# Kuntz-Lab/interactive-rate-tendons

Hardware: AMD Instinct MI355X
Metric: FK+collision checks/sec (3-tendon, 256^3 voxel env) (higher is better)
Workload: dtype f64

## Files before the change

interactive-rate-tendons_amd/_lib.py:

```python
import ctypes as C
import os
import subprocess

_PKG = os.path.dirname(os.path.abspath(__file__))
_ROOT = os.path.dirname(_PKG)
LIB_PATH = os.environ.get("TENDON_HIP_LIB") or os.path.join(_PKG, "libtendon_hip.so")
SRC_DIR = os.path.join(_PKG, "csrc")
HEADER = os.path.join(_ROOT, "include", "tendon_hip.h")

TR_OK, TR_ERR_INVALID_ARG, TR_ERR_OUT_OF_RANGE, TR_ERR_DOMAIN, TR_ERR_LENGTH, TR_ERR_RUNTIME, \
    TR_ERR_HIP, TR_ERR_UNSUPPORTED = range(8)

TR_FLAG_CONVERGED, TR_FLAG_LENGTH_OK, TR_FLAG_NO_SELFCOL, TR_FLAG_NO_VOXCOL, TR_FLAG_DOMAIN = 1, 2, 4, 8, 16
TR_CHECKER_BACKBONE, TR_CHECKER_SPHERES = 0, 1
TR_PROFILE_SLOTS = 6
PROFILE_SLOT_NAMES = ("fk_rk4_batch", "backbone_voxel_sweep", "cached_blocks_vs_grid", "edge_helpers", "fk_sweep_fused", "fk_verdict")

ABI_SYMBOLS = (
    "tr_create", "tr_destroy", "tr_last_error", "tr_state_size", "tr_num_points", "tr_device",
    "tr_home_lengths", "tr_set_grid", "tr_set_checker", "tr_grid_add_spheres", "tr_grid_add_capsules", "tr_grid_remove_interior", "tr_grid_dilate",
    "tr_grid_dilate_sphere", "tr_get_grid", "tr_reserve", "tr_reserve_edges", "tr_fk_batch", "tr_fk_batch_dev", "tr_fk_batch_retraction_dev",
    "tr_validate_shapes_retraction_dev",
    "tr_validate_batch", "tr_validate_batch_dev", "tr_validate_shapes_dev", "tr_validate_edges", "tr_validate_edges_indexed", "tr_validate_edges_last_valid",
    "tr_validate_edges_discrete",
# ... 54 lines not shown


class OutOfRange(TendonHipError, IndexError):
    status = TR_ERR_OUT_OF_RANGE


class DomainError(TendonHipError, ArithmeticError):
    status = TR_ERR_DOMAIN


class LengthError(TendonHipError, ValueError):
    status = TR_ERR_LENGTH


class HipError(TendonHipError):
    status = TR_ERR_HIP


class Unsupported(TendonHipError, NotImplementedError):
    status = TR_ERR_UNSUPPORTED


_EXC = {TR_ERR_INVALID_ARG: InvalidArgument, TR_ERR_OUT_OF_RANGE: OutOfRange, TR_ERR_DOMAIN: DomainError,
        TR_ERR_LENGTH: LengthError, TR_ERR_RUNTIME: TendonHipError, TR_ERR_HIP: HipError,
        TR_ERR_UNSUPPORTED: Unsupported}


HIPCC_FLAGS = ["--offload-arch=gfx950", "-O3", "-std=c++17", "-ffp-contract=off", "-fPIC"]
OBJ_DIR = os.path.join(SRC_DIR, "_obj")


def _units():
    fk_deps = ["fk_inst.hip", "fk_launch.hpp", "fk_kernel.hpp", "fk_retract_kernel.hpp", "fused_kernel.hpp", "verdict_kernel.hpp",
               "sweep_kernel.hpp", "sphere_kernel.hpp", "tr_types.hpp"]
    roadmap_deps = ["roadmap.hip", "roadmap_kernel.hpp", "search_kernel.hpp", "handback_feed.hpp", "roadmap_infra_host.inc", "roadmap_astar_host.inc",
                    "roadmap_components_host.inc", "roadmap_search_host.inc", "roadmap_solve_host.inc", "roadmap_tips_host.inc", "tipq_kernel.hpp"]
    fk_only = ["fk_inst.hip", "fk_kernel.hpp", "fk_retract_kernel.hpp", "cache_merge.hip", "sample.hip", "edge_queue_kernel.hpp"] + roadmap_deps
    main_deps = [f for f in os.listdir(SRC_DIR) if not f.startswith("_") and f not in fk_only]
    u = [("tendon_hip.o", "tendon_hip.hip", [], main_deps + [HEADER]),
         ("cache_merge.o", "cache_merge.hip", [], ["cache_merge.hip", "cache_merge.hpp"]),
         ("roadmap.o", "roadmap.hip", ["-pthread"], roadmap_deps + [HEADER]),
         ("sample.o", "sample.hip", [], ["sample.hip", "sample.hpp", "tr_types.hpp"])]
    q_deps = fk_deps + ["edge_queue_kernel.hpp", "edge_kernel.hpp"]
    for n in range(1, 9):
        for kind, tag in ((0, "u"), (1, "r"), (2, "f"), (3, "v"), (4, "w"), (5, "q")):
            u.append(("fk_%s%d.o" % (tag, n), "fk_inst.hip", ["-DTRK_INST_N=%d" % n, "-DTRK_INST_KIND=%d" % kind],
                      q_deps if kind == 5 else fk_deps))
    return u


def _sources():
    return [os.path.join(SRC_DIR, f) for f in sorted(os.listdir(SRC_DIR)) if not f.startswith("_")] + [HEADER]


def source_hash():
    import hashlib
    h = hashlib.sha1()
    for f in _sources():
        h.update(os.path.basename(f).encode())
        h.update(open(f, "rb").read())
    return h.hexdigest()[:16]


def build(force=False, verbose=False, jobs=None):
    stamp = LIB_PATH + ".srchash"
    want = source_hash()
    if not force and os.path.exists(LIB_PATH) and os.path.exists(stamp) and open(stamp).read().strip() == want:
# ... 189 lines not shown
```

interactive-rate-tendons_amd/csrc/edge_queue_kernel.hpp:

```cpp
#pragma once
#include "verdict_kernel.hpp"
#define TRK_EDGE_DEVICE_ONLY
#include "edge_kernel.hpp"

namespace trk {

__device__ __forceinline__ uint32_t eq_load(const uint32_t *p) { return __hip_atomic_load(p, __ATOMIC_RELAXED, __HIP_MEMORY_SCOPE_AGENT); }
__device__ __forceinline__ void eq_wait_vm() { asm volatile("s_waitcnt vmcnt(0)" ::: "memory"); }
__device__ __forceinline__ void eq_release() {
  eq_wait_vm();
  __builtin_amdgcn_fence(__ATOMIC_RELEASE, "agent");
  eq_wait_vm();
}
__device__ __forceinline__ void eq_acquire() {
  __builtin_amdgcn_fence(__ATOMIC_ACQUIRE, "agent");
  eq_wait_vm();
}
__device__ __forceinline__ int eq_bcast(int v) { return __builtin_amdgcn_readfirstlane(v); }
struct EqClock {
  unsigned long long t;
  __device__ __forceinline__ void start() { t = wall_clock64(); }
  __device__ __forceinline__ void lap(uint32_t *ctl, int word) {
    const unsigned long long n = wall_clock64();
    if (threadIdx.x == 0) __hip_atomic_fetch_add((unsigned long long *)(ctl + word), n - t, __ATOMIC_RELAXED, __HIP_MEMORY_SCOPE_AGENT);
// ... 150 lines not shown
    }
    ps.template sig_finish<false>();
    ps.finish();
    while (ps.qcount > 0) ps.flush();
    __syncthreads();
    LaneVerdict lv;
    int e2, h2, cnt2;
    {
      const VerdictArgs a = *va;
      const int sb = eq_stash_base(a.NM);
      e2 = VL_I(sb + lane); h2 = VL_I(sb + 64); cnt2 = VL_I(sb + 65);
      clk.t = (unsigned long long)VL_U(sb + 66) | ((unsigned long long)VL_U(sb + 67) << 32);
      lv = verdict_decide<N, false, true>(a, fl_, lane < cnt2);
    }
    const bool live2 = lane < cnt2;
    int zero2 = 0;
    asm volatile("" : "+s"(zero2));
    const EdgeQueueArgs &q2 = qa[zero2];
#ifdef TRK_EQ_TRACE
    const uint32_t tr_start = (uint32_t)clk.t;
    const unsigned long long tr_w0 = wall_clock64(), tr_c0 = (unsigned long long)clock64();
    { float x = (float)lane; for (int i = 0; i < 2000; i++) x = __builtin_fmaf(x, 1.0000001f, 0.5f); if (x == 12345.678f) asm volatile("s_nop 0"); }
    const unsigned long long tr_w1 = wall_clock64(), tr_c1 = (unsigned long long)clock64();
    const uint32_t tr_mhz = tr_w1 > tr_w0 ? (uint32_t)((tr_c1 - tr_c0) * 100ull / (tr_w1 - tr_w0)) : 0u;
#endif
    clk.lap(q2.ctl, EQ_T_FK);
#ifdef TRK_EQ_TRACE
    const uint32_t tr_fk = (uint32_t)clk.t;
#endif
    if (__any(lv.pending)) {
      __syncthreads();
      const double *st2 = q2.states + ((int64_t)h2 - (int64_t)blockIdx.x * 64) * K.state_size;
      const int64_t n2 = (int64_t)blockIdx.x * 64 + cnt2;
      fk_uniform_body<N, ROT, false, false>(st2, n2, q2.fb_ld, K, tab, steps, nsteps, q2.fb_out, NoPointHook(), nullptr, nullptr);
      __syncthreads();
      const FusedSweepArgs fa = *sa;
      bool exact = false;
      sweep_body<false>(q2.fb_in, n2, q2.fb_ld, fa.P, fa.CH, fa.NM, K, fa.g, fa.grid, fa.near_grid, 1, fa.debug, nullptr, nullptr, nullptr, &exact);
      __syncthreads();
      const uint32_t npend = (uint32_t)__popcll(__ballot(lv.pending));
      if (lane == 0) __hip_atomic_fetch_add(q2.ctl + EQ_PENDING, npend, __ATOMIC_RELAXED, __HIP_MEMORY_SCOPE_AGENT);
      if (lv.pending) lv.valid = exact;
      clk.lap(q2.ctl, EQ_T_EXACT);
    }

    if (live2 && !lv.valid) q2.edge_ok[e2] = 0u;
    eq_release();
    int old = 0;
    if (live2) old = __hip_atomic_fetch_add(q2.remaining + e2, -1, __ATOMIC_RELAXED, __HIP_MEMORY_SCOPE_AGENT);
    bool fin = live2 && old == 1;
    bool stop = false;
    EqClock sub = clk;
    sub.lap(q2.ctl, EQ_T_F0);
    if (__any(fin)) {
      eq_acquire();
      {
        const uint32_t nfin = (uint32_t)__popcll(__ballot(fin));
        if (lane == 0) __hip_atomic_fetch_add(q2.ctl + EQ_FINISHED, nfin, __ATOMIC_RELAXED, __HIP_MEMORY_SCOPE_AGENT);
      }
      int base_l = 0, ncand_l = 0;
      double rel_l = 0.0;
      if (fin && q2.edge_ok[e2] != 0u) {
        base_l = q2.lvl_base[e2]; ncand_l = q2.lvl_cnt[e2]; rel_l = q2.rel[e2];
        if (2 * ncand_l > EQ_MAX_CAND) {
          __hip_atomic_fetch_or(q2.ctl + EQ_FLAGS, EQF_DEEP, __ATOMIC_RELAXED, __HIP_MEMORY_SCOPE_AGENT);
          ncand_l = 0; stop = true;
        }
// ... 140 lines not shown
```

interactive-rate-tendons_amd/csrc/fk_kernel.hpp:

```cpp
#pragma once
#include <type_traits>
#include <hip/hip_runtime.h>
#include "tr_types.hpp"

namespace trk {

#ifndef TRK_NEWTON_STEPS
#define TRK_NEWTON_STEPS 1
#endif
__device__ __forceinline__ double fast_rcp(double x) {
  double y = __builtin_amdgcn_rcp(x);
  double e = __builtin_fma(-x, y, 1.0);
  y = __builtin_fma(e, y, y);
#if TRK_NEWTON_STEPS > 1
  e = __builtin_fma(-x, y, 1.0);
  y = __builtin_fma(e, y, y);
#endif
  return y;
}
__device__ __forceinline__ double fast_rsqrt(double x) {
  double y = __builtin_amdgcn_rsq(x);
  double hx = 0.5 * x;
  double t = __builtin_fma(-hx * y, y, 0.5);
  y = __builtin_fma(y, t, y);
#if TRK_NEWTON_STEPS > 1
  t = __builtin_fma(-hx * y, y, 0.5);
  y = __builtin_fma(y, t, y);
#endif
  return y;
}

template <int N, class Route>
__device__ __forceinline__ void strain_rates_routed(const double v[3], const double u[3], const double (&tau)[N],
                                                    Route &&route, const RobotK &K,
                                                    double dv[3], double du[3], double (&sdot)[N]) {
#pragma clang fp contract(fast)
  double Axx = K.ks0, Axy = 0, Axz = 0, Ayy = K.ks0, Ayz = 0, Azz = K.ks2, Z = 0;
  double B00 = 0, B01 = 0, B02 = 0, B10 = 0, B11 = 0, B12 = 0, B20 = 0, B21 = 0, B22 = 0, Q1 = 0, Q2 = 0;
  double Hxx = K.kb0, Hxy = 0, Hxz = 0, Hyy = K.kb0, Hyz = 0, Hzz = K.kb2;
  double ax = 0, ay = 0, az = 0, bx = 0, by = 0, bz = 0;
#pragma unroll
  for (int j = 0; j < N; j++) {
    double r6[6];
    route(j, r6);
    const double rx = r6[0], ry = r6[1];
    const double rdx = r6[2], rdy = r6[3];
    const double rddx = r6[4], rddy = r6[5];
    const double pdx = (v[0] + rdx) - u[2] * ry;
    const double pdy = (v[1] + rdy) + u[2] * rx;
    const double pdz = __builtin_fma(u[0], ry, __builtin_fma(-u[1], rx, v[2]));
    const double sxy = pdx * pdx + pdy * pdy, s2 = sxy + pdz * pdz;
    const double rs = fast_rsqrt(s2);
    sdot[j] = s2 * rs;
    const double cs2 = -tau[j] * rs;
    const double c = cs2 * (rs * rs);
    const double qx = c * pdx, qy = c * pdy, qz = c * pdz;
    Axx += qx * pdx; Axy += qx * pdy; Axz += qx * pdz; Ayy += qy * pdy; Ayz += qy * pdz; Azz += qz * pdz;
    Z += cs2;
    const double ez = rx * pdy - ry * pdx;
    const double gx = ry * qz, gy = -rx * qz, gz = c * ez;
    B00 += gx * pdx; B01 += gx * pdy; B02 += gx * pdz;
    B10 += gy * pdx; B11 += gy * pdy; B12 += gy * pdz;
    B20 += gz * pdx; B21 += gz * pdy; B22 += gz * pdz;
    Hxz += gx * ez; Hyz += gy * ez; Hzz += gz * ez;
    const double mxy = c * sxy, mx = mxy * rx, my = mxy * ry;
    Hxx -= my * ry; Hxy += mx * ry; Hyy -= mx * rx;
    const double t1 = cs2 * rx, t2 = cs2 * ry;
    Q1 += t1; Q2 += t2;
    Hzz -= t1 * rx; Hzz -= t2 * ry;
    const double hx = pdx + rdx, hy = pdy + rdy, hz = pdz;
    const double wx = __builtin_fma(u[1], hz, __builtin_fma(-u[2], hy, rddx));
    const double wy = __builtin_fma(u[2], hx, __builtin_fma(-u[0], hz, rddy));
    const double wz = u[0] * hy - u[1] * hx;
    const double pw = pdx * wx + pdy * wy + pdz * wz;
    const double aix = qx * pw - cs2 * wx, aiy = qy * pw - cs2 * wy, aiz = qz * pw - cs2 * wz;
    ax += aix; ay += aiy; az += aiz;
    bx += ry * aiz; by -= rx * aiz; bz += rx * aiy - ry * aix;
  }
#define TRK_FMA __builtin_fma
  B02 -= Q2; B12 += Q1; B20 += Q2; B21 -= Q1;
  const double svx = K.ks0 * v[0], svy = K.ks0 * v[1], svz = K.ks2 * (v[2] - 1.0);
  const double dku = K.dkb * u[2], w = TRK_FMA(-K.ks0, v[2], svz);
  const double cx = TRK_FMA(-u[1], dku, TRK_FMA(-v[1], w, -bx));
  const double cy = TRK_FMA(u[0], dku, TRK_FMA(v[0], w, -by));
  const double cz = -bz;
  const double dx = TRK_FMA(u[2], svy, TRK_FMA(-u[1], svz, -ax));
  const double dy = TRK_FMA(u[0], svz, TRK_FMA(-u[2], svx, -ay));
  const double dz = TRK_FMA(u[1], svx, TRK_FMA(-u[0], svy, -az));
  const double m00 = Axx - Z, m01 = Axy, m02 = Axz, m11 = Ayy - Z, m12 = Ayz, m22 = Azz - Z;
#ifndef TRK_SOLVE_SCHUR
  {
#pragma clang fp contract(off)
    const double n00 = Hxx, n01 = Hxy, n02 = Hxz, n11 = Hyy, n12 = Hyz, n22 = Hzz;
    const double p0 = m00;
    const double r0 = fast_rcp(p0);
    const double w10 = m01, l10 = w10 * r0;
    const double w20 = m02, l20 = w20 * r0;
    const double w30 = B00, l30 = w30 * r0;
    const double w40 = B10, l40 = w40 * r0;
    const double w50 = B20, l50 = w50 * r0;
    const double p1 = TRK_FMA(-l10, w10, m11);
    const double r1 = fast_rcp(p1);
// ... 46 lines not shown
  const double s00 = TRK_FMA(-T02, B02, TRK_FMA(-T01, B01, TRK_FMA(-T00, B00, Hxx)));
  const double s01 = TRK_FMA(-T02, B12, TRK_FMA(-T01, B11, TRK_FMA(-T00, B10, Hxy)));
  const double s02 = TRK_FMA(-T02, B22, TRK_FMA(-T01, B21, TRK_FMA(-T00, B20, Hxz)));
  const double s11 = TRK_FMA(-T12, B12, TRK_FMA(-T11, B11, TRK_FMA(-T10, B10, Hyy)));
  const double s12 = TRK_FMA(-T12, B22, TRK_FMA(-T11, B21, TRK_FMA(-T10, B20, Hyz)));
  const double s22 = TRK_FMA(-T22, B22, TRK_FMA(-T21, B21, TRK_FMA(-T20, B20, Hzz)));
  const double ex = TRK_FMA(-B02, yz, TRK_FMA(-B01, yy_, TRK_FMA(-B00, yx, cx)));
  const double ey = TRK_FMA(-B12, yz, TRK_FMA(-B11, yy_, TRK_FMA(-B10, yx, cy)));
  const double ez = TRK_FMA(-B22, yz, TRK_FMA(-B21, yy_, TRK_FMA(-B20, yx, cz)));
  const double g00 = TRK_FMA(s11, s22, -(s12 * s12)), g01 = TRK_FMA(s02, s12, -(s01 * s22)), g02 = TRK_FMA(s01, s12, -(s02 * s11));
  const double g11 = TRK_FMA(s00, s22, -(s02 * s02)), g12 = TRK_FMA(s01, s02, -(s00 * s12)), g22 = TRK_FMA(s00, s11, -(s01 * s01));
  const double isd = fast_rcp(TRK_FMA(s00, g00, TRK_FMA(s01, g01, s02 * g02)));
  du[0] = TRK_FMA(g00, ex, TRK_FMA(g01, ey, g02 * ez)) * isd;
  du[1] = TRK_FMA(g01, ex, TRK_FMA(g11, ey, g12 * ez)) * isd;
  du[2] = TRK_FMA(g02, ex, TRK_FMA(g12, ey, g22 * ez)) * isd;
  dv[0] = TRK_FMA(-T20, du[2], TRK_FMA(-T10, du[1], TRK_FMA(-T00, du[0], yx)));
  dv[1] = TRK_FMA(-T21, du[2], TRK_FMA(-T11, du[1], TRK_FMA(-T01, du[0], yy_)));
  dv[2] = TRK_FMA(-T22, du[2], TRK_FMA(-T12, du[1], TRK_FMA(-T02, du[0], yz)));
#endif
#undef TRK_FMA
}

template <int N>
__device__ __forceinline__ void strain_rates(const double v[3], const double u[3], const double (&tau)[N],
                                             const double *__restrict__ ri, const RobotK &K,
                                             double dv[3], double du[3], double (&sdot)[N]) {
  strain_rates_routed<N>(v, u, tau, [&](int j, double (&r6)[6]) {
#pragma unroll
    for (int q = 0; q < 6; q++) r6[q] = ri[6 * j + q];
  }, K, dv, du, sdot);
}

template <int N>
__device__ __forceinline__ void initial_bending(const double (&tau)[N], const double *__restrict__ rb,
                                                const RobotK &K, double v[3], double u[3], bool &converged) {
#pragma clang fp contract(off)
  v[0] = 0; v[1] = 0; v[2] = 1;
  u[0] = 0; u[1] = 0; u[2] = 0;
  bool done = false;
  for (int it = 0; it < 1000; ++it) {
    if (!__any(!done)) break;
    double Fx = 0, Fy = 0, Fz = 0, Lx = 0, Ly = 0, Lz = 0;
#pragma unroll
    for (int k = 0; k < N; k++) {
      const double rx = rb[6 * k + 0], ry = rb[6 * k + 1], rdx = rb[6 * k + 2], rdy = rb[6 * k + 3];
      double px = (-u[2] * ry) + rdx + v[0];
      double py = (u[2] * rx) + rdy + v[1];
      double pz = (u[0] * ry - u[1] * rx) + v[2];
      const double z = px * px + py * py + pz * pz;
      if (z > 0.0) { const double s = sqrt(z); px = px / s; py = py / s; pz = pz / s; }
      Fx -= tau[k] * px; Fy -= tau[k] * py; Fz -= tau[k] * pz;
      const double trx = tau[k] * rx, try_ = tau[k] * ry;
      Lx -= try_ * pz; Ly -= (-trx) * pz; Lz -= ((-try_) * px + trx * py);
    }
    const double nx = K.ks0 * v[0], ny = K.ks0 * v[1], nz = K.ks2 * (v[2] - 1);
    const double mx = K.kb0 * u[0], my = K.kb0 * u[1], mz = K.kb2 * u[2];
    const double e1 = (nx - Fx) * (nx - Fx) + (ny - Fy) * (ny - Fy) + (nz - Fz) * (nz - Fz);
    const double e2 = (mx - Lx) * (mx - Lx) + (my - Ly) * (my - Ly) + (mz - Lz) * (mz - Lz);
    const double residual = sqrt(e1 + e2);
    if (!done && residual < K.residual_threshold) done = true;
    const double vnx = K.iks0 * Fx, vny = K.iks0 * Fy, vnz = K.iks2 * Fz + 1;
    const double unx = K.ikb0 * Lx, uny = K.ikb0 * Ly, unz = K.ikb2 * Lz;
    if (!done) {
      const double dvn = sqrt((vnx - v[0]) * (vnx - v[0]) + (vny - v[1]) * (vny - v[1]) + (vnz - v[2]) * (vnz - v[2]));
      const double dun = sqrt((unx - u[0]) * (unx - u[0]) + (uny - u[1]) * (uny - u[1]) + (unz - u[2]) * (unz - u[2]));
      const double vn = sqrt(v[0] * v[0] + v[1] * v[1] + v[2] * v[2]);
// ... 96 lines not shown
    for (int q = 0; q < 3; q++) { av[q] += bw * dv[q]; au[q] += bw * du[q]; }
    if (st < 3) {
#pragma unroll
      for (int q = 0; q < 9; q++) sR[q] = R[q] + aw * dR[q];
#pragma unroll
      for (int q = 0; q < 3; q++) { sv[q] = v[q] + aw * dv[q]; su[q] = u[q] + aw * du[q]; }
    }
  }
#pragma unroll
  for (int q = 0; q < 9; q++) R[q] = __builtin_fma(b1, aR[q], R[q]);
#pragma unroll
  for (int q = 0; q < 3; q++) { v[q] = av[q]; u[q] = au[q]; }
}


template <int N>
struct FkLane {
  bool converged;
  double Li[N];
  double tip[3];
};

struct NoPointHook {
  __device__ __forceinline__ void begin(bool) const {}
  __device__ __forceinline__ void operator()(int, double, double, double) const {}
  __device__ __forceinline__ void tip_point(int, bool, bool, double, double, double, bool = true) const {}
};

template <class H, class = void> struct HookLiInLds { static constexpr int from = 1 << 30; };
template <class H> struct HookLiInLds<H, std::void_t<decltype(H::kLiInLdsFrom)>> { static constexpr int from = H::kLiInLdsFrom; };
template <class OnPoint> __host__ __device__ constexpr bool li_in_lds(int N) {
  return N >= HookLiInLds<std::remove_cv_t<std::remove_reference_t<OnPoint>>>::from && N <= 4;
}

template <int N, bool ROT, bool WRITE_R, bool WANT_L = true, class OnPoint = NoPointHook>
__device__ __forceinline__ void fk_uniform_body(
    const double *__restrict__ states, int64_t n, int64_t ld, const RobotK &K,
    const double *__restrict__ tab, const StepK *__restrict__ steps, int nsteps, const FkOut &out,
    OnPoint &&on_point = NoPointHook(), const int32_t *__restrict__ row_map = nullptr, FkLane<N> *lane_out = nullptr) {
#pragma clang fp contract(fast)
  const int64_t i = (int64_t)blockIdx.x * 64 + threadIdx.x;
  const bool live = i < n;
  const int64_t il = live ? i : (n - 1);
  const int64_t ic = row_map ? (int64_t)row_map[il] : il;
  const int S = K.state_size;
  double tau[N];
#pragma unroll
  for (int j = 0; j < N; j++) tau[j] = states[ic * S + j];
  constexpr bool kLiLds = li_in_lds<OnPoint>(N);
  double *li_lds = nullptr;
  if constexpr (kLiLds) {
    __shared__ double li_lds_store[N * 64];
    li_lds = li_lds_store;
#pragma unroll
    for (int j = 0; j < N; j++) li_lds[j * 64 + threadIdx.x] = 0.0;
  }
  double rc = 1.0, rs = 0.0, r22 = 1.0;
  if (ROT) {
    const double th = states[ic * S + N];
    rs = sin(th); rc = cos(th);
    r22 = (1.0 - rc) + rc;
  }

  double v[3], u[3];
  bool conv;
  initial_bending<N>(tau, tab, K, v, u, conv);
  on_point.begin(conv && live);

  double R[9] = {1, 0, 0, 0, 1, 0, 0, 0, 1};
  double p[3] = {0, 0, 0};
  double Lb = 0;
  double Li[N];
#pragma unroll
  for (int j = 0; j < N; j++) Li[j] = 0;

  auto store_point = [&](int j) {
    const int64_t o = (int64_t)j * ld + i;
    double x = p[0], y = p[1], z = p[2];
    if (ROT) { const double x2 = __builtin_fma(rc, x, -(rs * y)), y2 = __builtin_fma(rs, x, rc * y); x = x2; y = y2; z = r22 * z; }
    on_point(j, x, y, z);
    if (!live) return;
    if (out.px) { out.px[o] = x; out.py[o] = y; out.pz[o] = z; }
    if (WRITE_R) {
      const int64_t PS = (int64_t)K.n_points * ld;
#pragma unroll
      for (int c = 0; c < 3; c++) {
        double a = R[c * 3 + 0], b = R[c * 3 + 1], cc = R[c * 3 + 2];
        if (ROT) { const double a2 = rc * a - rs * b, b2 = rs * a + rc * b; a = a2; b = b2; cc = r22 * cc; }
        out.R[(c * 3 + 0) * PS + o] = a; out.R[(c * 3 + 1) * PS + o] = b; out.R[(c * 3 + 2) * PS + o] = cc;
      }
    }
  };
  store_point(0);

  for (int k = 0; k < nsteps; k++) {
    const double h = steps[k].h;
    const int obs = steps[k].obs;
    const double *__restrict__ rt = tab + (size_t)(1 + 3 * k) * (N * 6);
    const double hh = h * 0.5;
    const double b1 = h * (1.0 / 6.0), b2 = h * (1.0 / 3.0);
    double aR[9], av[3], au[3];
#pragma unroll
    for (int q = 0; q < 3; q++) { av[q] = v[q]; au[q] = u[q]; }
    double sR[9], sv[3], su[3];
    double qs[3], qm[3];
#pragma unroll
    for (int q = 0; q < 9; q++) sR[q] = R[q];
#pragma unroll
    for (int q = 0; q < 3; q++) { sv[q] = v[q]; su[q] = u[q]; }

#pragma unroll
    for (int st = 0; st < 4; st++) {
      const double *__restrict__ ri = rt + (st == 0 ? 0 : (st == 3 ? 2 : 1)) * (N * 6);
      const double bw = (st == 0 || st == 3) ? b1 : b2;
      const double aw = (st == 2) ? h : hh;
      double dv[3], du[3], sd[N];
      strain_rates<N>(sv, su, tau, ri, K, dv, du, sd);
      position_quadrature(st, sR, sv, b1, qs, qm, p);
      if (WANT_L && out.L) {
        const double v2 = sv[0] * sv[0] + sv[1] * sv[1] + sv[2] * sv[2];
        Lb += bw * (v2 * fast_rsqrt(v2));
      }
      if constexpr (kLiLds) {
#pragma unroll
        for (int j = 0; j < N; j++) li_lds[j * 64 + threadIdx.x] += bw * sd[j];
      } else {
#pragma unroll
        for (int j = 0; j < N; j++) Li[j] += bw * sd[j];
      }
      double dR[9];
      frame_rate(st, sR, su, dR, aR);
#pragma unroll
      for (int q = 0; q < 3; q++) { av[q] += bw * dv[q]; au[q] += bw * du[q]; }
      if (st < 3) {
#pragma unroll
        for (int q = 0; q < 9; q++) sR[q] = R[q] + aw * dR[q];
#pragma unroll
        for (int q = 0; q < 3; q++) { sv[q] = v[q] + aw * dv[q]; su[q] = u[q] + aw * du[q]; }
      }
    }
#pragma unroll
    for (int q = 0; q < 9; q++) R[q] = __builtin_fma(b1, aR[q], R[q]);
#pragma unroll
    for (int q = 0; q < 3; q++) { v[q] = av[q]; u[q] = au[q]; }
    if (obs >= 0) store_point(obs);
  }

  if constexpr (kLiLds) {
#pragma unroll
    for (int j = 0; j < N; j++) Li[j] = li_lds[j * 64 + threadIdx.x];
// ... 34 lines not shown
```

interactive-rate-tendons_amd/csrc/sweep_kernel.hpp:

```cpp
#pragma once
#include <hip/hip_runtime.h>
#include "tr_types.hpp"

#ifndef TRK_K2_PF
#define TRK_K2_PF 4
#endif

namespace trk {

struct V3 { double x, y, z; };

__device__ __forceinline__ double dot3(const V3 &a, const V3 &b) {
#pragma clang fp contract(off)
  return a.x * b.x + a.y * b.y + a.z * b.z;
}

__device__ __forceinline__ bool segment_aabox_intersect(const V3 &A, const V3 &B, const GridK &g) {
#pragma clang fp contract(off)
  const V3 AB = {B.x - A.x, B.y - A.y, B.z - A.z};
  const double len = sqrt(dot3(AB, AB)) / 2;
  const V3 U = {AB.x / (2 * len), AB.y / (2 * len), AB.z / (2 * len)};
  const V3 Ua = {fabs(U.x), fabs(U.y), fabs(U.z)};
  const V3 P = {(A.x + B.x) / 2 - (g.xmax + g.xmin) / 2, (A.y + B.y) / 2 - (g.ymax + g.ymin) / 2,
                (A.z + B.z) / 2 - (g.zmax + g.zmin) / 2};
// ... 214 lines not shown
#endif
constexpr int SIG_T = 8, SIG_LDS_STRIDE = 72, SIG_LDS_WORDS = SIG_T * SIG_LDS_STRIDE;
struct SigStage {
  int cur, mask;
  __device__ __forceinline__ void init() { cur = -1; mask = 0; }
  template <class Word>
  __device__ __forceinline__ void flush(Word &&W, uint32_t *__restrict__ sig, int64_t stride, int row_of, int first_row) {
    if (cur < 0) return;
    __syncthreads();
    const int lane = threadIdx.x, w = lane & (SIG_T - 1), sub = lane >> 3;
    const int j = cur * SIG_T + w;
#pragma unroll TRK_SIG_FLUSH_UNROLL
    for (int it = 0; it < 8; it++) {
      const int r = it * 8 + sub;
      const int ro = __shfl(row_of, r, 64), fr = __shfl(first_row, r, 64);
      const uint32_t v = W(w * SIG_LDS_STRIDE + r);
      if (((mask >> w) & 1) && ro >= 0 && j >= fr) sig[(int64_t)ro * stride + j] = v;
    }
    __syncthreads();
    cur = -1; mask = 0;
  }
  template <class Word>
  __device__ __forceinline__ void put(Word &&W, uint32_t *__restrict__ sig, int64_t stride, int row_of, int first_row, int row, bool on,
                                      uint32_t value) {
    const int tile = row >> 3;
    if (tile != cur) { flush(W, sig, stride, row_of, first_row); cur = tile; }
    if (on) W((row & (SIG_T - 1)) * SIG_LDS_STRIDE + (int)threadIdx.x) = value;
    mask |= 1 << (row & (SIG_T - 1));
  }
};

struct SignatureHook {
  static constexpr int kLiInLdsFrom = 3;
  const FusedSweepArgs *sa;
  int64_t n;
  bool any;
  SigStage st;
  __device__ __forceinline__ static uint32_t &word(int i) { extern __shared__ float lds[]; return ((uint32_t *)lds)[i]; }
  __device__ __forceinline__ int row_of() const { const int64_t i = (int64_t)blockIdx.x * 64 + threadIdx.x; return i < n ? (int)i : -1; }
  __device__ __forceinline__ void begin(bool) const {}
  __device__ __forceinline__ void operator()(int j, double x, double y, double z) {
    if (!any) return;
    int zero = 0;
    asm volatile("" : "+s"(zero));
    const FusedSweepArgs &a = sa[zero];
    st.put([](int i) -> uint32_t & { return word(i); }, a.sig, a.sig_stride, row_of(), 0, j, true, cell_signature(x, y, z, a.g));
  }
  __device__ __forceinline__ void finish() {
    if (!any) return;
    st.flush([](int i) -> uint32_t & { return word(i); }, sa->sig, sa->sig_stride, row_of(), 0);
  }
};

__device__ __forceinline__ bool exact_self_collision(const SweepIn &in, int64_t ic, int64_t ld, int P, int np,
                                                     bool act, double hmax, double r, bool brute) {
#pragma clang fp contract(off)
  const double consider = 3.0 * r;
  const double rsum = r + r;
  const double h_eff = hmax * (1.0 + 1e-9) + 1e-300;
  const double inv_h = 1.0 / h_eff;
  bool selfhit = false;
  act = act && np > 2;
  for (int a = 0; a < P - 3; ++a) {
    if (!__any(act && a < np - 3)) break;
    const bool act_a = act && a < np - 3;
    const int64_t oa = (int64_t)a * ld + ic;
// ... 439 lines not shown
```

interactive-rate-tendons_amd/csrc/tendon_hip.hip:

```cpp
#include <hip/hip_runtime.h>
#include <sched.h>

#include <algorithm>
#include <cfloat>
#include <cmath>
#include <cstdio>
#include <cstdlib>
#include <cstring>
#include <chrono>
#include <thread>
#include <ctime>
#include <limits>
#include <mutex>
#include <string>
#include <vector>

#include "../../include/tendon_hip.h"
#include "tr_types.hpp"
#include "fk_launch.hpp"
#include "sweep_kernel.hpp"
#include "sphere_kernel.hpp"
#include "verdict_kernel.hpp"
#include "edge_kernel.hpp"
#include "edge_plan.hpp"
#include "knn_kernel.hpp"
#include "cache_merge.hpp"
#include "env_kernel.hpp"
#include "sample.hpp"
#include "ik_kernel.hpp"

void tr_dev_cache_trim();
struct tr_ctx;
namespace { void ik_release(tr_ctx *c); }

namespace {

std::string g_create_error;

struct Workspace {
  int64_t ld = 0;
  double *px = nullptr, *py = nullptr, *pz = nullptr, *acc = nullptr;
  double *Li = nullptr;
  double *homeLi = nullptr;
  int32_t *np = nullptr;
  uint8_t *conv = nullptr;
  int64_t st_cap = 0;
  double *states = nullptr;
  uint64_t *bits = nullptr;
  double *tips = nullptr;
  uint8_t *flags = nullptr;
  double *L = nullptr;
  int32_t *npts = nullptr;
// ... 801 lines not shown
  c->C.assign(rb->C, rb->C + (size_t)N * rb->n_a);
  c->D.assign(rb->D, rb->D + (size_t)N * rb->n_m);
  c->max_tension.assign(rb->max_tension, rb->max_tension + N);
  for (int j = 0; j < N; j++) { K.min_len[j] = rb->min_length[j]; K.max_len[j] = rb->max_length[j]; }
  {
    const double ro2 = rb->ro * rb->ro, ri2 = rb->ri * rb->ri;
    const double I = (1.0 / 4.0) * M_PI * (ro2 * ro2 - ri2 * ri2);
    const double Ar = M_PI * (ro2 - ri2);
    const double J = 2 * I;
    const double Gmod = rb->E / (2 * (1 + rb->nu));
    K.kb0 = rb->E * I; K.kb2 = J * Gmod; K.dkb = K.kb2 - K.kb0;
    K.ikb0 = 1 / (rb->E * I); K.ikb2 = 1 / (J * Gmod);
    K.ks0 = Gmod * Ar; K.ks2 = rb->E * Ar;
    K.iks0 = 1 / (Gmod * Ar); K.iks2 = 1 / (rb->E * Ar);
  }
  c->t = t_range(0.0, rb->L, rb->dL);
  K.n_points = (int)c->t.size();
  std::vector<double> step_t;
  for (size_t j = 0; j + 1 < c->t.size(); j++) {
    double cur = c->t[j];
    const double tn = c->t[j + 1];
    bool any = false;
    while (tn - cur > DBL_EPSILON) {
      const double h = std::min(rb->dL, tn - cur);
      c->steps.push_back(StepK{h, -1, 0});
      step_t.push_back(cur);
      cur += h;
      any = true;
    }
    if (!any) { c->steps.push_back(StepK{0.0, -1, 0}); step_t.push_back(cur); }
    c->steps.back().obs = (int)j + 1;
  }
  const size_t ent = (size_t)N * 6;
  std::vector<double> tab((1 + 3 * c->steps.size()) * ent);
  routing_at(c, 0.0, tab.data());
  for (size_t k = 0; k < c->steps.size(); k++) {
    const double tk = step_t[k], h = c->steps[k].h;
    routing_at(c, tk, &tab[(1 + 3 * k + 0) * ent]);
    routing_at(c, tk + h * 0.5, &tab[(1 + 3 * k + 1) * ent]);
    routing_at(c, tk + h, &tab[(1 + 3 * k + 2) * ent]);
  }
  home_lengths(c, c->t, 0.0, K.home_Li);
  for (size_t k = 0; k < c->steps.size(); k++) if (c->steps[k].obs == 1) c->k_first = (int)k + 1;
  c->rows_one_step = (int)c->steps.size() - c->k_first == K.n_points - 2;
  for (size_t k = (size_t)c->k_first; k < c->steps.size() && c->rows_one_step; k++)
    if (c->steps[k].obs != (int)k - c->k_first + 2) c->rows_one_step = false;
  std::vector<double> hl(c->t.size() * (size_t)N);
  for (size_t q = 0; q < c->t.size(); q++)
    for (int j = 0; j < N; j++) {
      const double *Cj = &c->C[(size_t)j * rb->n_a], *Dj = &c->D[(size_t)j * rb->n_m];
      double Cdot[TRK_MAX_COEF] = {0}, Ddot[TRK_MAX_COEF] = {0};
      for (int k = 1; k < rb->n_a; k++) Cdot[k - 1] = k * Cj[k];
      for (int k = 1; k < rb->n_m; k++) Ddot[k - 1] = k * Dj[k];
      const double dd = poly_at(Ddot, rb->n_m, c->t[q]), dv = poly_at(Dj, rb->n_m, c->t[q]), cd = poly_at(Cdot, rb->n_a, c->t[q]);
      hl[q * N + j] = std::sqrt(dd * dd + (dv * dv) * (cd * cd) + 1);
    }
  PolyK poly{};
  for (int j = 0; j < N; j++) {
    for (int i = 0; i < rb->n_a; i++) poly.C[j][i] = c->C[(size_t)j * rb->n_a + i];
    for (int i = 0; i < rb->n_m; i++) poly.D[j][i] = c->D[(size_t)j * rb->n_m + i];
    const int rdeg = poly_degree(&c->D[(size_t)j * rb->n_m], rb->n_m), tdeg = poly_degree(&c->C[(size_t)j * rb->n_a], rb->n_a);
    poly.home_kind[j] = (rdeg == 0 && tdeg == 0) ? 0 : ((rdeg == 0 && tdeg == 1) ? 1 : 2);
    const double d0 = poly.D[j][0], c1 = rb->n_a > 1 ? poly.C[j][1] : 0.0;
    poly.helix_scale[j] = std::sqrt(1 + d0 * d0 * c1 * c1);
  }

  auto bail = [&](const char *what) { std::string m = what; tr_destroy(c); return fail(nullptr, TR_ERR_HIP, m); };
  if (hipMalloc((void **)&c->d_poly, sizeof(PolyK)) != hipSuccess) return bail("hipMalloc(poly)");
  if (hipMemcpy(c->d_poly, &poly, sizeof(PolyK), hipMemcpyHostToDevice) != hipSuccess) return bail("hipMemcpy(poly)");
  if (hipMalloc((void **)&c->d_tgrid, c->t.size() * sizeof(double)) != hipSuccess ||
      hipMalloc((void **)&c->d_hl, hl.size() * sizeof(double)) != hipSuccess) return bail("hipMalloc(tgrid)");
  if (hipMemcpy(c->d_tgrid, c->t.data(), c->t.size() * sizeof(double), hipMemcpyHostToDevice) != hipSuccess ||
      hipMemcpy(c->d_hl, hl.data(), hl.size() * sizeof(double), hipMemcpyHostToDevice) != hipSuccess) return bail("hipMemcpy(tgrid)");
  if (hipMalloc((void **)&c->d_tab, tab.size() * sizeof(double)) != hipSuccess) return bail("hipMalloc(tab)");
// ... 1090 lines not shown
```

interactive-rate-tendons_amd/csrc/verdict_kernel.hpp:

```cpp
#pragma once
#include "fk_kernel.hpp"
#define TRK_DEVICE_BODIES_ONLY
#include "sweep_kernel.hpp"
#include "sphere_kernel.hpp"

namespace trk {

struct VerdictHot {
  double box[6];
  double org[3], inv_d[3];
  const uint64_t *near_grid;
  int32_t Nb, rot_is_identity, P, CH;
  int32_t use_near;
  int32_t pad_;
};
static_assert(sizeof(VerdictHot) == 128, "one 128-byte block");

struct alignas(128) VerdictArgs {
  VerdictHot hot;
  int P, CH, NM, pad0_;
  uint32_t debug, pad1_;
  double box[6];
  GridK g;
  const uint64_t *grid, *near_grid;
// ... 27 lines not shown
#endif
template <bool SIG>
struct VLay {
  static constexpr int VQ = SIG ? TRK_SIG_VQ : 128;
  static constexpr int QE = 3 * 64;
  static constexpr int W0 = 2 * (QE + 6 * VQ);
  static constexpr int QOWNER = W0, OWNER_WORDS = SIG ? (VQ + 3) / 4 : VQ;
  static constexpr int CELL = QOWNER + OWNER_WORDS, INPREV = CELL + 3 * 64, HIT = INPREV + 64, DIST = HIT + 64, DELTA = DIST + 64, MS = DELTA + 64;
  static constexpr int NEARW = DELTA;
  __device__ static __forceinline__ int wrap(int i) {
    if constexpr ((VQ & (VQ - 1)) == 0) return i & (VQ - 1); else return i >= VQ ? i - VQ : i;
  }
  __device__ static __forceinline__ void set_owner(int slot, int lane) {
    if constexpr (SIG) ((uint8_t *)vlds)[4 * QOWNER + slot] = (uint8_t)lane; else ((uint32_t *)vlds)[QOWNER + slot] = (uint32_t)lane;
  }
  __device__ static __forceinline__ int owner(int slot) {
    if constexpr (SIG) return (int)((const uint8_t *)vlds)[4 * QOWNER + slot]; else return (int)((const uint32_t *)vlds)[QOWNER + slot];
  }
};
__host__ __device__ inline size_t verdict_lds_bytes(int NM, bool with_sig = false) {
  return (size_t)(with_sig ? VLay<true>::MS : VLay<false>::MS) * 4 + (size_t)4 * NM * 64 * sizeof(float) + (with_sig ? (size_t)SIG_LDS_WORDS * 4 : 0);
}

#define VL_D(i) (((double *)vlds)[(i)])
#define VL_U(i) (((uint32_t *)vlds)[(i)])
#define VL_I(i) (((int32_t *)vlds)[(i)])
#define VL_F(i) (((float *)vlds)[(i)])
#define VL_BARRIER() asm volatile("" ::: "memory")

template <bool SPH, bool SIG = false>
struct PointSweep {
  using Lay = VLay<SIG>;
  static constexpr int VQ = Lay::VQ;
  static constexpr int kLiInLdsFrom = (SIG && TRK_SIG_VQ > 88) ? (1 << 30) : 4;
  const VerdictArgs *va;
  float dn_prev;
  uint32_t sph_state;
  int qhead, qcount;
  int P, CH, NM, Kl, ms_next, ms_k;
  SigStage sigst;
  int sig_row_of, sig_first_row;
  int sig_row0, sig_cnt;
  bool active;

  __device__ __forceinline__ int sig_own_row() const { const int l = (int)threadIdx.x; return l < sig_cnt ? sig_row0 + l : -1; }
  __device__ __forceinline__ void sig_rows_of_launch(int64_t n) {
    const int64_t r0 = (int64_t)blockIdx.x * 64, left = n - r0;
    sig_row0 = (int)r0; sig_cnt = left >= 64 ? 64 : (left > 0 ? (int)left : 0);
  }
  __device__ __forceinline__ void sig_put(const VerdictArgs &a, int row, bool on, uint32_t value, int row_of, int first_row) {
    const int base = Lay::MS + 4 * NM * 64;
    sigst.put([base](int i) -> uint32_t & { return VL_U(base + i); }, a.sig, a.sig_stride, row_of, first_row, row, on, value);
  }
  template <bool RETRACT>
  __device__ __forceinline__ void sig_finish() {
    if constexpr (SIG) {
      const VerdictArgs &a = args();
      const int base = Lay::MS + 4 * NM * 64;
      sigst.flush([base](int i) -> uint32_t & { return VL_U(base + i); }, a.sig, a.sig_stride, RETRACT ? sig_row_of : sig_own_row(),
                  RETRACT ? sig_first_row : 0);
    }
  }

  __device__ __forceinline__ void begin(bool on) { active = on; }

  __device__ __forceinline__ const VerdictArgs &args() const {
    int zero = 0;
// ... 525 lines not shown
```

profiles/kbench.hip:

```cpp
#include <hip/hip_runtime.h>
#include <algorithm>
#include <cmath>
#include <cstdio>
#include <cstdlib>
#include <vector>
#include "tr_types.hpp"
#include "fk_kernel.hpp"
#ifdef KB_VERDICT
#include "verdict_kernel.hpp"
#ifdef KB_SIG
constexpr bool kSig = true;
#else
constexpr bool kSig = false;
#endif
#endif

#ifndef KB_N
#define KB_N 3
#endif
#ifndef KB_LOG2
#define KB_LOG2 20
#endif
#ifndef KB_REPS
#define KB_REPS 7
// ... 13 lines not shown

#define CK(x) do { hipError_t e_ = (x); if (e_ != hipSuccess) { std::fprintf(stderr, "%s: %s\n", #x, hipGetErrorString(e_)); return 1; } } while (0)

static void routing_at(int N, const double C[][3], const double D[][3], double t, double *out) {
  for (int j = 0; j < N; j++) {
    const double th = C[j][0] + C[j][1] * t + C[j][2] * t * t, th1 = C[j][1] + 2 * C[j][2] * t, th2 = 2 * C[j][2];
    const double rho = D[j][0] + D[j][1] * t + D[j][2] * t * t, rho1 = D[j][1] + 2 * D[j][2] * t, rho2 = 2 * D[j][2];
    const double sa = std::sin(th), ca = std::cos(th);
    double *o = out + 6 * j;
    o[0] = rho * sa; o[1] = rho * ca;
    o[2] = rho1 * sa + rho * (ca * th1);
    o[3] = rho1 * ca + rho * (-sa * th1);
    o[4] = rho2 * sa + 2 * rho1 * (ca * th1) - rho * (sa * th1 * th1) + rho * (ca * th2);
    o[5] = rho2 * ca + 2 * rho1 * (-sa * th1) - rho * (ca * th1 * th1) + rho * (-sa * th2);
  }
}

int main() {
  constexpr int N = KB_N;
  const double L = 0.2, dL = L / 128, ro = 0.01, ri = 0.0, E = 2.1e6, nu = 0.3;
  double C[8][3] = {}, D[8][3] = {};
  if (N == 3) for (int k = 0; k < 3; k++) { C[k][0] = 2 * M_PI * k / 3; C[k][1] = 5.0; D[k][0] = 0.01; }
  else {
    const double c1[4] = {3.0, -2.0, 4.0, -5.0}, c2[4] = {10.0, 15.0, -12.0, 8.0}, d1[4] = {-0.01, 0.005, 0.0, -0.005};
    for (int k = 0; k < N; k++) { C[k][0] = M_PI * k / 2; C[k][1] = c1[k % 4]; C[k][2] = c2[k % 4]; D[k][0] = 0.01; D[k][1] = d1[k % 4]; }
  }
  RobotK K{};
  {
    const double ro2 = ro * ro, ri2 = ri * ri, I = 0.25 * M_PI * (ro2 * ro2 - ri2 * ri2), Ar = M_PI * (ro2 - ri2), J = 2 * I, G = E / (2 * (1 + nu));
    K.kb0 = E * I; K.kb2 = J * G; K.dkb = K.kb2 - K.kb0; K.ikb0 = 1 / K.kb0; K.ikb2 = 1 / K.kb2; K.ks0 = G * Ar; K.ks2 = E * Ar; K.iks0 = 1 / K.ks0; K.iks2 = 1 / K.ks2;
  }
  K.residual_threshold = 5e-6; K.radius = 0.015; K.L = L; K.dL = dL; K.n_tendons = N; K.n_a = 3; K.n_m = 3; K.state_size = N; K.n_points = 129;
  std::vector<StepK> steps;
  std::vector<double> tab((1 + 3 * 128) * N * 6);
  routing_at(N, C, D, 0.0, tab.data());
  for (int k = 0; k < 128; k++) {
    const double tk = k * dL;
    steps.push_back(StepK{dL, k + 1, 0});
    for (int q = 0; q < 3; q++) routing_at(N, C, D, tk + 0.5 * q * dL, &tab[(size_t)(1 + 3 * k + q) * N * 6]);
  }
#ifdef KB_COUNT
  const int64_t n = KB_COUNT;
#else
  const int64_t n = (int64_t)1 << KB_LOG2;
#endif
  std::vector<double> st((size_t)n * N);
  unsigned long long lcg = 88172645463325252ull;
  const double tmax = N == 3 ? 10.0 : 20.0;
  for (auto &x : st) { lcg = lcg * 6364136223846793005ull + 1442695040888963407ull; x = tmax * (double)(lcg >> 11) * (1.0 / 9007199254740992.0); }
  double *d_st, *d_tab, *d_tips; StepK *d_steps;
  CK(hipMalloc(&d_st, st.size() * 8)); CK(hipMalloc(&d_tab, tab.size() * 8)); CK(hipMalloc(&d_tips, (size_t)n * 24)); CK(hipMalloc(&d_steps, steps.size() * sizeof(StepK)));
  CK(hipMemcpy(d_st, st.data(), st.size() * 8, hipMemcpyHostToDevice)); CK(hipMemcpy(d_tab, tab.data(), tab.size() * 8, hipMemcpyHostToDevice));
  CK(hipMemcpy(d_steps, steps.data(), steps.size() * sizeof(StepK), hipMemcpyHostToDevice));
  hipEvent_t a, b; CK(hipEventCreate(&a)); CK(hipEventCreate(&b));
#ifdef KB_VERDICT
  trk::VerdictArgs va{};
  va.P = 129; va.CH = (int)std::lround(2.0 * K.radius / dL); va.NM = (128 + va.CH - 1) / va.CH + 1;
  GridK &g = va.g;
  g.xmin = g.ymin = g.zmin = -0.25; g.xmax = g.ymax = g.zmax = 0.25; g.N = 256; g.Nb = 64; g.rot_is_identity = 1;
  g.dx = g.dy = g.dz = 0.5 / 256; g.inv_dx = g.inv_dy = g.inv_dz = 1 / g.dx;
  for (int q = 0; q < 9; q++) g.inv_rot[q] = (q % 4 == 0) ? 1.0 : 0.0;
  for (int q = 0; q < 3; q++) { va.box[2 * q] = -0.25 + 1e-6 * 0.5; va.box[2 * q + 1] = 0.25 - 1e-6 * 0.5; }
  uint64_t *d_grid, *d_bits; int32_t *d_fb; uint32_t *d_fbc; trk::VerdictArgs *d_va;
  CK(hipMalloc(&d_grid, (size_t)64 * 64 * 64 * 8 * 2)); CK(hipMemset(d_grid, 0, (size_t)64 * 64 * 64 * 8 * 2));
  CK(hipMalloc(&d_bits, (size_t)((n + 63) / 64) * 8)); CK(hipMalloc(&d_fb, (size_t)n * 4)); CK(hipMalloc(&d_fbc, 4)); CK(hipMemset(d_fbc, 0, 4));
  va.grid = d_grid; va.near_grid = d_grid + 64 * 64 * 64; va.valid_bits = d_bits; va.fb_list = d_fb; va.fb_count = d_fbc;
  va.radius = K.radius;
  uint32_t *d_sig = nullptr;
  if (kSig) { va.sig_stride = (129 + 15) / 16 * 16; CK(hipMalloc(&d_sig, (size_t)n * va.sig_stride * 4)); va.sig = d_sig; }
  for (int j = 0; j < N; j++) { va.min_len[j] = K.min_len[j] = -1.0; va.max_len[j] = K.max_len[j] = 1.0; va.home_Li[j] = K.home_Li[j] = L; }
  va.finish_hot();
  CK(hipMalloc(&d_va, sizeof(va))); CK(hipMemcpy(d_va, &va, sizeof(va), hipMemcpyHostToDevice));
  const size_t lds = trk::verdict_lds_bytes(va.NM, kSig);
// ... 35 lines not shown
```

Before: 134.8 million.

## Precompute tendon routing products and stream them through an LDS ring

Routing-dependent products (rx², rx·ry, ry², rx²+ry²) are now precomputed on the host and appended to the routing table. In the RK4 loop they are prefetched one step ahead into registers and staged into a shared-memory slot, so each stage reads them instead of recomputing them. The Hessian accumulation is also rewritten as explicit FMAs using these products. The trade-off is extra LDS use and more register pressure for the prefetch buffer, which can cut occupancy; the ring is disabled for some hooks or for N=4, and the FMA regrouping may change rounding slightly.

```diff
diff --git a/interactive-rate-tendons_amd/_lib.py b/interactive-rate-tendons_amd/_lib.py
--- a/interactive-rate-tendons_amd/_lib.py
+++ b/interactive-rate-tendons_amd/_lib.py
@@ -110,7 +110,7 @@
 
 def _units():
     fk_deps = ["fk_inst.hip", "fk_launch.hpp", "fk_kernel.hpp", "fk_retract_kernel.hpp", "fused_kernel.hpp", "verdict_kernel.hpp",
-               "sweep_kernel.hpp", "sphere_kernel.hpp", "tr_types.hpp"]
+               "sweep_kernel.hpp", "sphere_kernel.hpp", "tr_types.hpp", "routing_products.hpp"]
     roadmap_deps = ["roadmap.hip", "roadmap_kernel.hpp", "search_kernel.hpp", "handback_feed.hpp", "roadmap_infra_host.inc", "roadmap_astar_host.inc",
                     "roadmap_components_host.inc", "roadmap_search_host.inc", "roadmap_solve_host.inc", "roadmap_tips_host.inc", "tipq_kernel.hpp"]
     fk_only = ["fk_inst.hip", "fk_kernel.hpp", "fk_retract_kernel.hpp", "cache_merge.hip", "sample.hip", "edge_queue_kernel.hpp"] + roadmap_deps
diff --git a/interactive-rate-tendons_amd/csrc/edge_queue_kernel.hpp b/interactive-rate-tendons_amd/csrc/edge_queue_kernel.hpp
--- a/interactive-rate-tendons_amd/csrc/edge_queue_kernel.hpp
+++ b/interactive-rate-tendons_amd/csrc/edge_queue_kernel.hpp
@@ -206,7 +206,7 @@
       __syncthreads();
       const double *st2 = q2.states + ((int64_t)h2 - (int64_t)blockIdx.x * 64) * K.state_size;
       const int64_t n2 = (int64_t)blockIdx.x * 64 + cnt2;
-      fk_uniform_body<N, ROT, false, false>(st2, n2, q2.fb_ld, K, tab, steps, nsteps, q2.fb_out, NoPointHook(), nullptr, nullptr);
+      fk_uniform_body<N, ROT, false, false>(st2, n2, q2.fb_ld, K, tab, steps, nsteps, q2.fb_out, NoPointHookNoSlot4(), nullptr, nullptr);
       __syncthreads();
       const FusedSweepArgs fa = *sa;
       bool exact = false;
diff --git a/interactive-rate-tendons_amd/csrc/fk_kernel.hpp b/interactive-rate-tendons_amd/csrc/fk_kernel.hpp
--- a/interactive-rate-tendons_amd/csrc/fk_kernel.hpp
+++ b/interactive-rate-tendons_amd/csrc/fk_kernel.hpp
@@ -2,6 +2,7 @@
 #include <type_traits>
 #include <hip/hip_runtime.h>
 #include "tr_types.hpp"
+#include "routing_products.hpp"
 
 namespace trk {
 
@@ -30,10 +31,14 @@
   return y;
 }
 
-template <int N, class Route>
+struct ProductsInLane {
+  __device__ __forceinline__ void operator()(int, const double (&r6)[6], double (&p4)[kProductCols]) const { routing_products(r6[0], r6[1], p4); }
+};
+template <int N, class Route, class Products = ProductsInLane>
 __device__ __forceinline__ void strain_rates_routed(const double v[3], const double u[3], const double (&tau)[N],
                                                     Route &&route, const RobotK &K,
-                                                    double dv[3], double du[3], double (&sdot)[N]) {
+                                                    double dv[3], double du[3], double (&sdot)[N],
+                                                    Products &&products = ProductsInLane()) {
 #pragma clang fp contract(fast)
   double Axx = K.ks0, Axy = 0, Axz = 0, Ayy = K.ks0, Ayz = 0, Azz = K.ks2, Z = 0;
   double B00 = 0, B01 = 0, B02 = 0, B10 = 0, B11 = 0, B12 = 0, B20 = 0, B21 = 0, B22 = 0, Q1 = 0, Q2 = 0;
@@ -50,6 +55,9 @@
     const double pdy = (v[1] + rdy) + u[2] * rx;
     const double pdz = __builtin_fma(u[0], ry, __builtin_fma(-u[1], rx, v[2]));
     const double sxy = pdx * pdx + pdy * pdy, s2 = sxy + pdz * pdz;
+    double p4[kProductCols];
+    products(j, r6, p4);
+    const double xx = p4[0], xy = p4[1], yy = p4[2], rr = p4[3];
     const double rs = fast_rsqrt(s2);
     sdot[j] = s2 * rs;
     const double cs2 = -tau[j] * rs;
@@ -63,11 +71,10 @@
     B10 += gy * pdx; B11 += gy * pdy; B12 += gy * pdz;
     B20 += gz * pdx; B21 += gz * pdy; B22 += gz * pdz;
     Hxz += gx * ez; Hyz += gy * ez; Hzz += gz * ez;
-    const double mxy = c * sxy, mx = mxy * rx, my = mxy * ry;
-    Hxx -= my * ry; Hxy += mx * ry; Hyy -= mx * rx;
-    const double t1 = cs2 * rx, t2 = cs2 * ry;
-    Q1 += t1; Q2 += t2;
-    Hzz -= t1 * rx; Hzz -= t2 * ry;
+    const double mxy = c * sxy;
+    Hxx = __builtin_fma(-mxy, yy, Hxx); Hxy = __builtin_fma(mxy, xy, Hxy); Hyy = __builtin_fma(-mxy, xx, Hyy);
+    Q1 = __builtin_fma(cs2, rx, Q1); Q2 = __builtin_fma(cs2, ry, Q2);
+    Hzz = __builtin_fma(-cs2, rr, Hzz);
     const double hx = pdx + rdx, hy = pdy + rdy, hz = pdz;
     const double wx = __builtin_fma(u[1], hz, __builtin_fma(-u[2], hy, rddx));
     const double wy = __builtin_fma(u[2], hx, __builtin_fma(-u[0], hz, rddy));
@@ -180,6 +187,47 @@
 }
 
 template <int N>
+__device__ __forceinline__ void strain_rates_lds(const double v[3], const double u[3], const double (&tau)[N],
+                                                 const double *__restrict__ ri, const double *slot, int po, const RobotK &K,
+                                                 double dv[3], double du[3], double (&sdot)[N]) {
+  const double *pr = (const double *)((const char *)slot + po);
+  strain_rates_routed<N>(v, u, tau, [&](int j, double (&r6)[6]) {
+#pragma unroll
+    for (int q = 0; q < 6; q++) r6[q] = ri[6 * j + q];
+  }, K, dv, du, sdot, [&](int j, const double (&)[6], double (&p4)[kProductCols]) {
+#pragma unroll
+    for (int q = 0; q < kProductCols; q++) p4[q] = pr[kProductCols * j + q];
+  });
+}
+
+template <int N>
+struct ProductRing {
+  static constexpr int ROW = N * kProductCols, CH = routing_products_fetches(N);
+  double *slot;
+  const double *__restrict__ prod;
+  double pend[CH];
+  __device__ __forceinline__ static double *storage() {
+    __shared__ __attribute__((aligned(16))) double product_slot_store[64 * CH];
+    return product_slot_store;
+  }
+  __device__ __forceinline__ void fetch(int k) {
+    const double *__restrict__ src = prod + routing_products_fetch_begin(k, N);
+#pragma unroll
+    for (int c = 0; c < CH; c++) pend[c] = src[c * 64 + threadIdx.x];
+  }
+  __device__ __forceinline__ void put() {
+#pragma unroll
+    for (int c = 0; c < CH; c++) slot[c * 64 + threadIdx.x] = pend[c];
+  }
+  __device__ __forceinline__ void begin(const double *__restrict__ tab, int nsteps) {
+    slot = storage();
+    prod = tab + routing_products_offset(nsteps, N);
+    fetch(0);
+    put();
+  }
+};
+
+template <int N>
 __device__ __forceinline__ void initial_bending(const double (&tau)[N], const double *__restrict__ rb,
                                                 const RobotK &K, double v[3], double u[3], bool &converged) {
 #pragma clang fp contract(off)
@@ -342,6 +390,15 @@
 template <class OnPoint> __host__ __device__ constexpr bool li_in_lds(int N) {
   return N >= HookLiInLds<std::remove_cv_t<std::remove_reference_t<OnPoint>>>::from && N <= 4;
 }
+template <class H, class = void> struct HookProductSlot { static constexpr bool at(int) { return true; } };
+template <class H> struct HookProductSlot<H, std::void_t<decltype(H::product_slot(0))>> { static constexpr bool at(int N) { return H::product_slot(N); } };
+struct NoPointHookNoSlot4 : NoPointHook { static constexpr bool product_slot(int N) { return N != 4; } };
+template <class OnPoint> __host__ __device__ constexpr bool products_in_lds(int N) {
+#ifdef TRK_NO_PRODUCT_RING
+  return false;
+#endif
+  return HookProductSlot<std::remove_cv_t<std::remove_reference_t<OnPoint>>>::at(N);
+}
 
 template <int N, bool ROT, bool WRITE_R, bool WANT_L = true, class OnPoint = NoPointHook>
 __device__ __forceinline__ void fk_uniform_body(
@@ -376,6 +433,9 @@
   bool conv;
   initial_bending<N>(tau, tab, K, v, u, conv);
   on_point.begin(conv && live);
+  constexpr bool kRing = products_in_lds<OnPoint>(N);
+  ProductRing<N> pring;
+  if constexpr (kRing) pring.begin(tab, nsteps);
 
   double R[9] = {1, 0, 0, 0, 1, 0, 0, 0, 1};
   double p[3] = {0, 0, 0};
@@ -407,6 +467,7 @@
     const double h = steps[k].h;
     const int obs = steps[k].obs;
     const double *__restrict__ rt = tab + (size_t)(1 + 3 * k) * (N * 6);
+    if constexpr (kRing) pring.fetch(k + 1);
     const double hh = h * 0.5;
     const double b1 = h * (1.0 / 6.0), b2 = h * (1.0 / 3.0);
     double aR[9], av[3], au[3];
@@ -425,7 +486,13 @@
       const double bw = (st == 0 || st == 3) ? b1 : b2;
       const double aw = (st == 2) ? h : hh;
       double dv[3], du[3], sd[N];
-      strain_rates<N>(sv, su, tau, ri, K, dv, du, sd);
+      if constexpr (kRing) {
+        const int po = (st == 0 ? 0 : (st == 3 ? 2 : 1)) * ProductRing<N>::ROW * (int)sizeof(double);
+        strain_rates_lds<N>(sv, su, tau, ri, pring.slot, po, K, dv, du, sd);
+        if (st == 3) pring.put();
+      } else {
+        strain_rates<N>(sv, su, tau, ri, K, dv, du, sd);
+      }
       position_quadrature(st, sR, sv, b1, qs, qm, p);
       if (WANT_L && out.L) {
         const double v2 = sv[0] * sv[0] + sv[1] * sv[1] + sv[2] * sv[2];
diff --git a/interactive-rate-tendons_amd/csrc/routing_products.hpp b/interactive-rate-tendons_amd/csrc/routing_products.hpp
--- /dev/null
+++ b/interactive-rate-tendons_amd/csrc/routing_products.hpp
@@ -0,0 +1,41 @@
+#pragma once
+#include <cstddef>
+
+#if defined(__HIPCC__) || defined(__CUDACC__)
+#define TRK_RP_HD __host__ __device__ __forceinline__
+#else
+#define TRK_RP_HD inline
+#endif
+
+namespace trk {
+
+constexpr int kProductCols = 4;
+
+TRK_RP_HD void routing_products(double rx, double ry, double (&p)[kProductCols]) {
+#if defined(__clang__)
+#pragma clang fp contract(off)
+#endif
+  const double xx = rx * rx, xy = rx * ry, yy = ry * ry;
+  p[0] = xx; p[1] = xy; p[2] = yy; p[3] = xx + yy;
+}
+
+constexpr size_t routing_products_offset(int nsteps, int N) { return (size_t)(1 + 3 * nsteps) * (size_t)N * 6; }
+constexpr int routing_products_fetches(int N) { return (3 * N * kProductCols + 63) / 64; }
+constexpr size_t routing_products_fetch_begin(int k, int N) { return (size_t)(1 + 3 * k) * (size_t)N * kProductCols; }
+constexpr size_t routing_products_doubles(int nsteps, int N) {
+  return routing_products_fetch_begin(nsteps, N) + (size_t)64 * routing_products_fetches(N);
+}
+constexpr size_t routing_table_doubles(int nsteps, int N) { return routing_products_offset(nsteps, N) + routing_products_doubles(nsteps, N); }
+
+inline void fill_routing_products(double *tab, int nsteps, int N) {
+  double *prod = tab + routing_products_offset(nsteps, N);
+  const size_t rows = (size_t)(1 + 3 * nsteps) * (size_t)N, total = routing_products_doubles(nsteps, N);
+  for (size_t r = 0; r < rows; r++) {
+    double p[kProductCols];
+    routing_products(tab[6 * r + 0], tab[6 * r + 1], p);
+    for (int q = 0; q < kProductCols; q++) prod[kProductCols * r + q] = p[q];
+  }
+  for (size_t i = rows * kProductCols; i < total; i++) prod[i] = 0.0;
+}
+
+}
diff --git a/interactive-rate-tendons_amd/csrc/sweep_kernel.hpp b/interactive-rate-tendons_amd/csrc/sweep_kernel.hpp
--- a/interactive-rate-tendons_amd/csrc/sweep_kernel.hpp
+++ b/interactive-rate-tendons_amd/csrc/sweep_kernel.hpp
@@ -270,6 +270,7 @@
 
 struct SignatureHook {
   static constexpr int kLiInLdsFrom = 3;
+  static constexpr bool product_slot(int) { return false; }
   const FusedSweepArgs *sa;
   int64_t n;
   bool any;
diff --git a/interactive-rate-tendons_amd/csrc/tendon_hip.hip b/interactive-rate-tendons_amd/csrc/tendon_hip.hip
--- a/interactive-rate-tendons_amd/csrc/tendon_hip.hip
+++ b/interactive-rate-tendons_amd/csrc/tendon_hip.hip
@@ -18,6 +18,7 @@
 #include "../../include/tendon_hip.h"
 #include "tr_types.hpp"
 #include "fk_launch.hpp"
+#include "routing_products.hpp"
 #include "sweep_kernel.hpp"
 #include "sphere_kernel.hpp"
 #include "verdict_kernel.hpp"
@@ -885,7 +886,7 @@
     c->steps.back().obs = (int)j + 1;
   }
   const size_t ent = (size_t)N * 6;
-  std::vector<double> tab((1 + 3 * c->steps.size()) * ent);
+  std::vector<double> tab(trk::routing_table_doubles((int)c->steps.size(), N));
   routing_at(c, 0.0, tab.data());
   for (size_t k = 0; k < c->steps.size(); k++) {
     const double tk = step_t[k], h = c->steps[k].h;
@@ -893,6 +894,7 @@
     routing_at(c, tk + h * 0.5, &tab[(1 + 3 * k + 1) * ent]);
     routing_at(c, tk + h, &tab[(1 + 3 * k + 2) * ent]);
   }
+  trk::fill_routing_products(tab.data(), (int)c->steps.size(), N);
   home_lengths(c, c->t, 0.0, K.home_Li);
   for (size_t k = 0; k < c->steps.size(); k++) if (c->steps[k].obs == 1) c->k_first = (int)k + 1;
   c->rows_one_step = (int)c->steps.size() - c->k_first == K.n_points - 2;
diff --git a/interactive-rate-tendons_amd/csrc/verdict_kernel.hpp b/interactive-rate-tendons_amd/csrc/verdict_kernel.hpp
--- a/interactive-rate-tendons_amd/csrc/verdict_kernel.hpp
+++ b/interactive-rate-tendons_amd/csrc/verdict_kernel.hpp
@@ -83,7 +83,8 @@
 struct PointSweep {
   using Lay = VLay<SIG>;
   static constexpr int VQ = Lay::VQ;
-  static constexpr int kLiInLdsFrom = (SIG && TRK_SIG_VQ > 88) ? (1 << 30) : 4;
+  static constexpr int kLiInLdsFrom = (SIG && TRK_SIG_VQ > 88) ? (1 << 30) : 3;
+  static constexpr bool product_slot(int N) { return N != 4; }
   const VerdictArgs *va;
   float dn_prev;
   uint32_t sph_state;
diff --git a/profiles/kbench.hip b/profiles/kbench.hip
--- a/profiles/kbench.hip
+++ b/profiles/kbench.hip
@@ -69,13 +69,14 @@
   }
   K.residual_threshold = 5e-6; K.radius = 0.015; K.L = L; K.dL = dL; K.n_tendons = N; K.n_a = 3; K.n_m = 3; K.state_size = N; K.n_points = 129;
   std::vector<StepK> steps;
-  std::vector<double> tab((1 + 3 * 128) * N * 6);
+  std::vector<double> tab(trk::routing_table_doubles(128, N));
   routing_at(N, C, D, 0.0, tab.data());
   for (int k = 0; k < 128; k++) {
     const double tk = k * dL;
     steps.push_back(StepK{dL, k + 1, 0});
     for (int q = 0; q < 3; q++) routing_at(N, C, D, tk + 0.5 * q * dL, &tab[(size_t)(1 + 3 * k + q) * N * 6]);
   }
+  trk::fill_routing_products(tab.data(), 128, N);
 #ifdef KB_COUNT
   const int64_t n = KB_COUNT;
 #else
```

Result: slower. 133.3 million (-1.1%).
